# FanmingL/Recurrent-Offpolicy-RL

Hardware: AMD Instinct MI355X
Metric: env-steps/sec trained (higher is better)
Workload: dtype f32; 1 GPU; smamba_s32_c16_b2_nln SAC-REDQ update, B=64/GPU, T=1024, D=256 (configs[1]; N=8: configs[3]); row_length=1043, obs=17, act=6, critic=efc-8, global_rows=64, parallelism=dp1

## Files before the change

include/resel_hip.h:

```cpp
#ifndef RESEL_HIP_H
#define RESEL_HIP_H

#include <stddef.h>
#include <stdint.h>

#ifdef __cplusplus
extern "C" {
#endif

#define RESEL_OK 0
#define RESEL_EINVAL (-1)
#define RESEL_ELAUNCH (-2)

typedef void* resel_stream_t;

int resel_abi_version(void);
const char* resel_build_info(void);

enum {
    RESEL_PROF_SSCAN_FWD = 0, RESEL_PROF_SSCAN_BWD = 1, RESEL_PROF_ATTN_FWD = 2, RESEL_PROF_ATTN_DQ = 3, RESEL_PROF_ATTN_DKV = 4,
    RESEL_PROF_LINREC_REAL_FWD = 5, RESEL_PROF_LINREC_REAL_BWD = 6, RESEL_PROF_LINREC_COMPLEX_FWD = 7, RESEL_PROF_LINREC_COMPLEX_BWD = 8,
    RESEL_PROF_GRU_FWD = 9, RESEL_PROF_GRU_BWD = 10, RESEL_PROF_CONV_FWD = 11, RESEL_PROF_CONV_BWD = 12, RESEL_PROF_GEMM = 13,
    RESEL_PROF_SSCAN_FWD_LOCAL = 14, RESEL_PROF_SSCAN_BWD_LOCAL = 15,
    RESEL_PROF_NSLOTS = 16
// ... 230 lines not shown
#define RESEL_CATEGORICAL_MAX_ACTIONS 4096
int resel_categorical_step(const float* logits, int64_t ld_logits, const float* u, float floor, float* logp, int64_t ld_logp,
                           float* mode, float* sample, int64_t ld_idx, int M, int A, resel_stream_t stream);

#define RESEL_TMAZE_STATE_WORDS 8
typedef struct { int32_t corridor_length, oracle_length, episode_length; double goal_reward, penalty, distract_reward; } resel_tmaze_cfg_t;
int resel_tmaze_step(resel_tmaze_cfg_t cfg, int init, const float* action, int64_t ld_action, const int32_t* goals, int64_t ld_goals,
                     const int32_t* n_episodes, int J, int32_t* env_state, double* ret_acc, double* ep_ret, int32_t* ep_len,
                     int64_t ld_ep, float* in_block, int64_t ld_in, int A, int32_t* flags, int B, resel_stream_t stream);

typedef struct { int32_t state, last_state, last_action, action, next_state, reward, logp, mask, start, done, reward_input, timeout; } resel_collect_layout_t;
int resel_tmaze_collect_step(resel_tmaze_cfg_t cfg, resel_collect_layout_t lay, int init, const float* action, int64_t ld_action,
                             const int32_t* goal, int32_t* env_state, double* ret_acc, float* traj, int T_cap, int64_t ld_row,
                             int max_episode_steps, float* in_block, int64_t ld_in, int A, int B, resel_stream_t stream);

int resel_categorical_fwd(const float* logits, float floor, float* logp, float* probs, float* mode, int M, int A, resel_stream_t stream);
int resel_categorical_bwd(const float* logits, float floor, const float* dlogp, const float* dprobs, float* dlogits, int M, int A,
                          resel_stream_t stream);
int resel_discrete_value(const float* q, const int32_t* subset, int m, const float* logp, const float* log_alpha, float* v,
                         int E, int M, int A, resel_stream_t stream);
int resel_q_taken_loss_fwd(const float* q, const float* action, const float* y, const float* mask, float* out2, void* workspace,
                           int E, int M, int A, resel_stream_t stream);
int resel_q_taken_loss_bwd(const float* q, const float* action, const float* y, const float* mask, const float* g, float* dq,
                           int E, int M, int A, resel_stream_t stream);
int resel_discrete_actor_loss_fwd(const float* logp, const float* q, const float* mask, const float* log_alpha, float* out2,
                                  void* workspace, int E, int M, int A, int reduce_min, resel_stream_t stream);
int resel_discrete_actor_loss_bwd(const float* logp, const float* q, const float* mask, const float* log_alpha, const float* g,
                                  float* dlogp, float* dq, int E, int M, int A, int reduce_min, resel_stream_t stream);

size_t resel_atb_workspace_bytes(int64_t K, int Wd, int Nd);
int resel_atb(const float* wide, int64_t ldw, int Wd, const float* narrow, int64_t ldn, int Nd, float* out, int transposed,
              void* workspace, int64_t K, resel_stream_t stream);

#ifdef __cplusplus
}
#endif
#endif
```

recurrent-offpolicy-rl_amd/csrc/skinny_gemm.hip:

```cpp
#include "resel_common.h"

namespace {
using namespace resel;

typedef float f32x16 __attribute__((ext_vector_type(16)));

__device__ __forceinline__ int acc_row(int r, int half) { return (r >> 2) * 8 + half * 4 + (r & 3); }

template <int NT>
__global__ __launch_bounds__(256) void atb_kernel(const float* __restrict__ Wm, int64_t ldw, int Wd, const float* __restrict__ Nm,
                                                  int64_t ldn, int Nd, float* __restrict__ part, int64_t K, int rows_per,
                                                  int transposed) {
    const int lane = threadIdx.x & 63, wave = threadIdx.x >> 6;
    const int half = lane >> 5, col = lane & 31;
    const int wb = blockIdx.y * 512 + wave * 128;
    if (wb >= Wd) return;
    const int64_t k0 = (int64_t)blockIdx.x * rows_per;
    const int64_t k1 = k0 + rows_per < K ? k0 + rows_per : K;
    f32x16 acc[4][NT];
#pragma unroll
    for (int e = 0; e < 4; ++e)
#pragma unroll
        for (int t = 0; t < NT; ++t)
#pragma unroll
            for (int r = 0; r < 16; ++r) acc[e][t][r] = 0.f;
    const int wc = wb + 4 * col;
    const bool w_ok = wc < Wd;
    bool n_ok[NT];
#pragma unroll
    for (int t = 0; t < NT; ++t) n_ok[t] = 32 * t + col < Nd;
    constexpr int UN = NT == 1 ? 8 : 4;
    for (int64_t k = k0; k < k1; k += 2 * UN) {
// ... 2 lines not shown
#pragma unroll
        for (int u = 0; u < UN; ++u) {
            const int64_t kr = k + 2 * u + half;
            const bool ok = kr < k1;
            a[u] = (ok && w_ok) ? ld4(Wm + kr * ldw + wc) : make_float4(0.f, 0.f, 0.f, 0.f);
#pragma unroll
            for (int t = 0; t < NT; ++t) b[u][t] = (ok && n_ok[t]) ? Nm[kr * ldn + 32 * t + col] : 0.f;
        }
#pragma unroll
        for (int u = 0; u < UN; ++u)
#pragma unroll
            for (int t = 0; t < NT; ++t) {
                acc[0][t] = __builtin_amdgcn_mfma_f32_32x32x2f32(a[u].x, b[u][t], acc[0][t], 0, 0, 0);
                acc[1][t] = __builtin_amdgcn_mfma_f32_32x32x2f32(a[u].y, b[u][t], acc[1][t], 0, 0, 0);
                acc[2][t] = __builtin_amdgcn_mfma_f32_32x32x2f32(a[u].z, b[u][t], acc[2][t], 0, 0, 0);
                acc[3][t] = __builtin_amdgcn_mfma_f32_32x32x2f32(a[u].w, b[u][t], acc[3][t], 0, 0, 0);
            }
    }
    float* dst = part + (int64_t)blockIdx.x * Wd * Nd;
#pragma unroll
    for (int e = 0; e < 4; ++e)
#pragma unroll
        for (int t = 0; t < NT; ++t) {
            const int n = 32 * t + col;
            if (n >= Nd) continue;
#pragma unroll
            for (int r = 0; r < 16; ++r) {
                const int w = wb + 4 * acc_row(r, half) + e;
                if (w < Wd) dst[transposed ? (int64_t)n * Wd + w : (int64_t)w * Nd + n] = acc[e][t][r];
            }
        }
}

inline int pick_ksplit(int64_t K, int Wd, int Nd) {
    int64_t ks = (int64_t)(16 << 20) / ((int64_t)Wd * Nd * 4);
    if (ks > 512) ks = 512;
    if (ks < 32) ks = 32;
    if (ks > (K + 1) / 2) ks = (K + 1) / 2;
    return (int)(ks < 1 ? 1 : ks);
}

}

extern "C" {

size_t resel_atb_workspace_bytes(int64_t K, int Wd, int Nd) {
    return (size_t)pick_ksplit(K, Wd, Nd) * Wd * Nd * sizeof(float);
}

int resel_atb(const float* wide, int64_t ldw, int Wd, const float* narrow, int64_t ldn, int Nd, float* out, int transposed,
              void* workspace, int64_t K, resel_stream_t stream) {
    if (!wide || !narrow || !out || !workspace || K <= 0 || Wd <= 0 || Nd <= 0) return RESEL_EINVAL;
    if (Nd > 96 || (Wd & 3) || (ldw & 3) || !aligned16(wide)) return RESEL_EINVAL;
    const int ks = pick_ksplit(K, Wd, Nd);
    int rows_per = (int)((K + ks - 1) / ks);
    rows_per += rows_per & 1;
    const int nsplit = (int)((K + rows_per - 1) / rows_per);
    const dim3 grid(nsplit, (Wd + 511) / 512), block(256);
    hipStream_t s = (hipStream_t)stream;
    float* part = (float*)workspace;
    const int NT = (Nd + 31) / 32;
    switch (NT) {
        case 1: hipLaunchKernelGGL(atb_kernel<1>, grid, block, 0, s, wide, ldw, Wd, narrow, ldn, Nd, part, K, rows_per, transposed); break;
        case 2: hipLaunchKernelGGL(atb_kernel<2>, grid, block, 0, s, wide, ldw, Wd, narrow, ldn, Nd, part, K, rows_per, transposed); break;
        default: hipLaunchKernelGGL(atb_kernel<3>, grid, block, 0, s, wide, ldw, Wd, narrow, ldn, Nd, part, K, rows_per, transposed); break;
    }
    launch_colsum(part, (int64_t)Wd * Nd, nsplit, Wd * Nd, out, s);
    return launch_status();
}

}
```

recurrent-offpolicy-rl_amd/offpolicy_rnn/hip/_lib.py:

```python
import ctypes
import os
from ctypes import c_float, c_int, c_int64, c_size_t, c_uint64, c_void_p

_HERE = os.path.dirname(os.path.abspath(__file__))
LIB_PATH = os.environ.get('RESEL_HIP_LIBRARY') or os.path.join(_HERE, 'libresel_hip.so')
ABI_VERSION = 11
_lib = None

P, I, L, F, S, U = c_void_p, c_int, c_int64, c_float, c_void_p, c_uint64
E = ctypes.c_uint

RESET_MAX_SEGS, RESET_MAX_COUNTERS = 16, 8


class ResetSeg(ctypes.Structure):
    _fields_ = [('base', c_void_p), ('row_stride', c_int64), ('width', ctypes.c_int32)]


class ResetSegs(ctypes.Structure):
    _fields_ = [('seg', ResetSeg * RESET_MAX_SEGS)]


class ResetCounters(ctypes.Structure):
    _fields_ = [('pos', c_void_p * RESET_MAX_COUNTERS)]
# ... 72 lines not shown
    'resel_soft_update': (c_int, [P, P, F, L, S]),
    'resel_adamw_flat': (c_int, [P, P, P, P, L, P, P, P, I, F, F, F, I, P, S]),
    'resel_adamw_flat_bc': (c_int, [P, P, P, P, L, P, P, P, I, F, F, F, F, F, P, S]),
    'resel_adamw_flat_dev': (c_int, [P, P, P, P, L, P, P, P, I, F, F, F, P, P, S]),
    'resel_sumsq_workspace_bytes': (c_size_t, [L]),
    'resel_sumsq': (c_int, [P, L, P, P, S]),
    'resel_bias_act_fwd': (c_int, [P, P, L, I, L, I, S]),
    'resel_bias_act_bwd_workspace_bytes': (c_size_t, [L, I, L]),
    'resel_bias_act_bwd': (c_int, [P, L, P, L, P, P, P, L, I, L, I, P, E, S]),
    'resel_ensemble_head_fwd': (c_int, [P, P, P, P, P, L, I, L, S]),
    'resel_ensemble_head_bwd_workspace_bytes': (c_size_t, [L, I, L]),
    'resel_ensemble_head_bwd': (c_int, [P, P, P, P, P, P, P, L, I, L, P, E, S]),
    'resel_gemm_f32_workspace_bytes': (c_size_t, [I, I, I, I]),
    'resel_gemm_f32': (c_int, [P, L, L, I, P, L, L, I, P, L, I, P, L, L, P, I, I, I, I, I, S]),
    'resel_gemm_f32x': (c_int, [P, L, L, I, P, L, L, I, P, L, I, P, L, L, P, I, I, I, I, I, P, P, P, E, S]),
    'resel_amax_segments': (c_int, [P, P, P, I, P, E, S]),
    'resel_amax_state_bytes': (c_size_t, []),
    'resel_amax': (c_int, [P, L, L, I, I, I, P, E, P, S]),
    'resel_gemm_f32_fused_supported': (c_int, [I, I, I, I, L, L]),
    'resel_gemm_f32_fused_workspace_bytes': (c_size_t, [I, I, I, I, I]),
    'resel_gemm_f32_dact': (c_int, [P, L, L, I, P, L, L, I, P, L, L, P, L, L, P, P, I, I, I, I, P, P, P, E, S]),
    'resel_gemm_f32_head': (c_int, [P, L, L, I, P, L, L, I, P, L, P, L, P, P, L, L, P, P, I, I, I, I, P, P, P, E, S]),
    'resel_amax_check': (c_int, [P, L, L, I, I, I, P, P, I, S]),
    'resel_gemm_bf16_workspace_bytes': (c_size_t, [I, I, I]),
    'resel_gemm_bf16': (c_int, [P, L, I, I, P, L, I, I, P, P, L, I, P, I, I, I, S]),
    'resel_colsum_bf16_workspace_bytes': (c_size_t, [I, I]),
    'resel_colsum_bf16': (c_int, [P, L, I, I, P, P, S]),
    'resel_gather_trajs': (c_int, [P, I, L, P, I, I, I, I, I, I, I, I, I, P, I, P, S]),
    'resel_gather_trajs_sel': (c_int, [P, I, L, P, I, I, I, I, I, I, I, I, I, P, I, P, I, P, S]),
    'resel_mamba_conv_step': (c_int, [P, L, P, L, P, L, L, L, I, P, P, P, I, I, I, I, S]),
    'resel_selective_state_update': (c_int, [P, L, P, L, P, P, L, P, P, P, P, P, L, P, I, I, I, I, S]),
    'resel_atb_workspace_bytes': (c_size_t, [L, I, I]),
    'resel_atb': (c_int, [P, L, I, P, L, I, P, I, P, L, S]),
    'resel_attn_decode': (c_int, [P, L, P, P, I, P, P, F, I, I, I, I, S]),
    'resel_attn_decode_rows': (c_int, [P, L, P, P, P, P, F, I, I, I, I, S]),
    'resel_step_state_reset': (c_int, [P, I, ResetSegs, I, ResetCounters, I, S]),
    'resel_categorical_step': (c_int, [P, L, P, F, P, L, P, P, L, I, I, S]),
    'resel_tmaze_step': (c_int, [TMazeCfg, I, P, L, P, L, P, I, P, P, P, P, L, P, L, I, P, I, S]),
    'resel_tmaze_collect_step': (c_int, [TMazeCfg, CollectLayout, I, P, L, P, P, P, P, I, L, I, P, L, I, I, S]),
    'resel_categorical_fwd': (c_int, [P, F, P, P, P, I, I, S]),
    'resel_categorical_bwd': (c_int, [P, F, P, P, P, I, I, S]),
    'resel_discrete_value': (c_int, [P, P, I, P, P, P, I, I, I, S]),
    'resel_q_taken_loss_fwd': (c_int, [P, P, P, P, P, P, I, I, I, S]),
    'resel_q_taken_loss_bwd': (c_int, [P, P, P, P, P, P, I, I, I, S]),
    'resel_discrete_actor_loss_fwd': (c_int, [P, P, P, P, P, P, I, I, I, I, S]),
    'resel_discrete_actor_loss_bwd': (c_int, [P, P, P, P, P, P, P, I, I, I, I, S]),
}


class ReselHipUnavailable(RuntimeError):
    pass


def lib():
    global _lib
    if _lib is not None:
        return _lib
    if not os.path.exists(LIB_PATH):
        raise ReselHipUnavailable(
            f'RESeL-HIP: {LIB_PATH} not found. The MI355X kernels are the only implementation of the hot path; '
            f'build them with `python -c "import __graft_entry__ as g; g.build()"` (or `make -C recurrent-offpolicy-rl_amd/csrc`).')
    handle = ctypes.CDLL(LIB_PATH)
    for name, (res, args) in SIGNATURES.items():
        fn = getattr(handle, name, None)
        if fn is None:
            raise ReselHipUnavailable(f'RESeL-HIP: symbol {name} missing from {LIB_PATH} (stale build?)')
# ... 13 lines not shown
```

recurrent-offpolicy-rl_amd/offpolicy_rnn/hip/ops.py:

```python
import ctypes
import os
from typing import Optional

import torch

from ._lib import check, lib


def _need_cuda(name, *ts):
    for t in ts:
        if t is not None and not t.is_cuda:
            raise RuntimeError(f'RESeL-HIP: {name} needs CUDA tensors (got a {t.device} tensor); the HIP kernels are the '
                               f'only implementation of this op - there is no CPU fallback.')


def _p(t: Optional[torch.Tensor]):
    return None if t is None else ctypes.c_void_p(t.data_ptr())


if hasattr(torch._C, '_cuda_getCurrentRawStream') and hasattr(torch._C, '_cuda_getDevice'):
    def _stream():
        return ctypes.c_void_p(torch._C._cuda_getCurrentRawStream(torch._C._cuda_getDevice()))
else:
    def _stream():
# ... 57 lines not shown
        SSCAN_TIME_SEGMENTS, amax_out, epoch, _stream()), 'selective_scan_fwd')


def _sscan_bwd(Bsz, L, u, delta, z, A, Bm, Cm, D, delta_bias, start, dout, ck, du, ddelta, dz, dB, dC, dA, dD, dbias, softplus,
               amax_dz=None, amax_ddelta=None, epoch=0):
    Di, N = A.shape
    ws = _ws(lib().resel_selective_scan_bwd_workspace_bytes(Bsz, L, Di, N, SSCAN_TIME_SEGMENTS), u.device)
    check(lib().resel_selective_scan_bwd(
        _p(u), u.stride(-2), _p(delta), delta.stride(-2), _p(z), 0 if z is None else z.stride(-2), _p(A),
        _p(Bm), Bm.stride(-2), _p(Cm), Cm.stride(-2), _p(D), _p(delta_bias), _p(start),
        _p(dout), dout.stride(-2), _p(ck),
        _p(du), du.stride(-2), _p(ddelta), ddelta.stride(-2), _p(dz), 0 if dz is None else dz.stride(-2),
        _p(dB), dB.stride(-2), _p(dC), dC.stride(-2), _p(dA), _p(dD), _p(dbias), _p(ws),
        Bsz, L, Di, N, softplus, SSCAN_TIME_SEGMENTS, amax_dz, amax_ddelta, epoch, _stream()), 'selective_scan_bwd')


def _conv_fwd(Bsz, L, x, w, bias, mask, y, act, amax_y=None, epoch=0):
    Di, K = w.shape
    check(lib().resel_causal_conv1d_fwd(_p(x), x.stride(-2), _p(w), _p(bias), _p(mask), _p(y), y.stride(-2), Bsz, L, Di, K, act,
                                        amax_y, epoch, _stream()), 'causal_conv1d_fwd')


def _conv_bwd(Bsz, L, x, w, bias, mask, dy, dy2, dx, dw, db, act, amax_dx=None, epoch=0):
    Di, K = w.shape
    ws = _ws(lib().resel_causal_conv1d_bwd_workspace_bytes(Bsz, L, Di, K), x.device)
    check(lib().resel_causal_conv1d_bwd2(_p(x), x.stride(-2), _p(w), _p(bias), _p(mask), _p(dy), dy.stride(-2),
                                         _p(dy2), 0 if dy2 is None else dy2.stride(-2), _p(dx), dx.stride(-2), _p(dw), _p(db), _p(ws),
                                         Bsz, L, Di, K, act, amax_dx, epoch, _stream()), 'causal_conv1d_bwd')


class SelectiveScanFn(torch.autograd.Function):

    @staticmethod
    def forward(ctx, u, delta, A, Bm, Cm, D, z, delta_bias, start, delta_softplus, return_last_state):
        _need_cuda('selective_scan', u, delta, A, Bm, Cm)
        u, delta, Bm, Cm = _tok_major(u), _tok_major(delta), _tok_major(Bm), _tok_major(Cm)
        z = None if z is None else _tok_major(z)
        A = A.float().contiguous()
        D = None if D is None else D.float().contiguous()
        delta_bias = None if delta_bias is None else delta_bias.float().contiguous()
        Bsz, L, Di = u.shape
        N = A.shape[1]
        start = _flags(start, Bsz, L)
        out = torch.empty(Bsz, L, Di, dtype=torch.float32, device=u.device)
        need_grad = any(ctx.needs_input_grad)
        ck = None
        if need_grad:
            ck = _ws(lib().resel_selective_scan_ckpt_bytes(Bsz, L, Di, N), u.device)
        last = torch.empty(Bsz, Di, N, dtype=torch.float32, device=u.device) if return_last_state else None
        _sscan_fwd(Bsz, L, u, delta, z, A, Bm, Cm, D, delta_bias, start, out, ck, last, int(bool(delta_softplus)))
        ctx.save_for_backward(u, delta, A, Bm, Cm, D, z, delta_bias, start, ck)
        ctx.softplus = bool(delta_softplus)
        if return_last_state:
            ctx.mark_non_differentiable(last)
            return out, last
        return out

    @staticmethod
    def backward(ctx, dout, *_):
        u, delta, A, Bm, Cm, D, z, delta_bias, start, ck = ctx.saved_tensors
        Bsz, L, Di = u.shape
        N = A.shape[1]
        dout = _tok_major(dout)
        dev = u.device
        du = torch.empty(Bsz, L, Di, dtype=torch.float32, device=dev)
        ddelta = torch.empty_like(du)
        dz = torch.empty_like(du) if z is not None else None
        dB = torch.empty(Bsz, L, N, dtype=torch.float32, device=dev)
        dC = torch.empty_like(dB)
        dA = torch.empty(Di, N, dtype=torch.float32, device=dev)
        dD = torch.empty(Di, dtype=torch.float32, device=dev) if D is not None else None
        dbias = torch.empty(Di, dtype=torch.float32, device=dev) if delta_bias is not None else None
        _sscan_bwd(Bsz, L, u, delta, z, A, Bm, Cm, D, delta_bias, start, dout, ck, du, ddelta, dz, dB, dC, dA, dD, dbias, int(ctx.softplus))
        return du, ddelta, dA, dB, dC, dD, dz, dbias, None, None, None


def selective_scan_tm(u, delta, A, Bm, Cm, D=None, z=None, delta_bias=None, start=None, delta_softplus=True,
                      return_last_state=False):
    return SelectiveScanFn.apply(u, delta, A, Bm, Cm, D, z, delta_bias, start, delta_softplus, return_last_state)


def selective_scan_fn(u, delta, A, B, C, start, D=None, z=None, delta_bias=None, delta_softplus=False,
                      return_last_state=False):
    tm = lambda t: None if t is None else t.transpose(1, 2)
    st = None if start is None else start[:, 0, :]
    res = selective_scan_tm(tm(u), tm(delta), A, tm(B), tm(C), D, tm(z), delta_bias, st, delta_softplus, return_last_state)
    if return_last_state:
        return res[0].transpose(1, 2), res[1]
    return res.transpose(1, 2)




class MambaInnerFn(torch.autograd.Function):

    @staticmethod
    def forward(ctx, x, in_w, conv_w, conv_b, xproj_w, dt_w, dt_b, A_log, D, out_w, mask, start):
        _need_cuda('mamba_inner', x, in_w, conv_w, xproj_w, dt_w, A_log, out_w)
        Bsz, L, Dm = x.shape
        Di, N = A_log.shape
        R = dt_w.shape[1]
        K = conv_w.shape[-1]
        M = Bsz * L
        x2 = x.reshape(M, Dm)
        maskf, startf = _flags(mask, Bsz, L), _flags(start, Bsz, L)
        xz = mm_nt(x2, in_w)
        ctx.ax = amax_of(x2)
        cw = conv_w.reshape(Di, K).contiguous()
        xc = torch.empty(M, Di, dtype=torch.float32, device=x.device)
        track = amax_tracking() and M * Di >= (1 << 20)
        h_xc, p_xc, e_xc = _slot_args(track, x.device)
        _conv_fwd(Bsz, L, xz, cw, conv_b, maskf, xc, 1, p_xc, e_xc)
        tag_amax(xc, h_xc)
        x_dbl = mm_nt(xc, xproj_w)
        if R < 32 <= R + 2 * N and os.environ.get('RESEL_DT_PAD', '1') != '0' and gemm_split() == 2:
            w32 = place_blocks(Di, 32, [(0, 0)], dt_w.detach())
            dt = gemm_f32(x_dbl[:, :32], w32, True, True, dt_b, GEMM_SOFTPLUS, amax_a=amax_of(x_dbl), amax_b=weight_amax(dt_w))
        else:
            dt = gemm_f32(x_dbl[:, :R], dt_w, True, True, dt_b, GEMM_SOFTPLUS)
        A = A_log.float().contiguous()
        need_grad = any(ctx.needs_input_grad)
        ck = _ws(lib().resel_selective_scan_ckpt_bytes(Bsz, L, Di, N), x.device) if need_grad else None
        y = torch.empty(M, Di, dtype=torch.float32, device=x.device)
        h_y, p_y, e_y = _slot_args(track, x.device)
        _sscan_fwd(Bsz, L, xc, dt, xz[:, Di:], A, x_dbl[:, R:R + N], x_dbl[:, R + N:], D, None, startf, y, ck, None, 6, p_y, e_y)
        tag_amax(y, h_y)
        out = mm_nt(y, out_w)
        ctx.handles = keep_handles(ctx.ax, h_xc, h_y)
        ctx.save_for_backward(x2, in_w, cw, conv_b, xproj_w, dt_w, dt_b, A, D, out_w, maskf, startf, xz, xc, x_dbl, dt, y, ck)
        ctx.dims = (Bsz, L, Dm, Di, N, R, K, conv_w.shape)
        return out.view(Bsz, L, -1)

    @staticmethod
    def backward(ctx, dout):
        (x2, in_w, cw, conv_b, xproj_w, dt_w, dt_b, A, D, out_w, maskf, startf, xz, xc, x_dbl, dt, y, ck) = ctx.saved_tensors
        Bsz, L, Dm, Di, N, R, K, cw_shape = ctx.dims
        M = Bsz * L
        dev = x2.device
        do2 = dout.reshape(M, -1)
        if not do2.is_contiguous():
            do2 = do2.contiguous()
        ax, h_xc, h_y = live_handles(ctx.handles)
        d_out_w = wgrad(do2, y, amax_x=h_y)
        dy = mm_nn(do2, out_w)
        dxz = torch.empty(M, 2 * Di, dtype=torch.float32, device=dev)
        dx_dbl = torch.empty(M, R + 2 * N, dtype=torch.float32, device=dev)
        dxc = torch.empty(M, Di, dtype=torch.float32, device=dev)
        ddt = torch.empty(M, Di, dtype=torch.float32, device=dev)
        dA = torch.empty(Di, N, dtype=torch.float32, device=dev)
        dD = torch.empty(Di, dtype=torch.float32, device=dev)
        ddt_b = torch.empty(Di, dtype=torch.float32, device=dev)
        track = amax_tracking() and M * Di >= (1 << 20)
        h_dxz, p_dxz, e_b = _slot_args(track, dev)
        h_ddt, p_ddt, _ = _slot_args(track, dev)
        _sscan_bwd(Bsz, L, xc, dt, xz[:, Di:], A, x_dbl[:, R:R + N], x_dbl[:, R + N:], D, None, startf, dy, ck,
                   dxc, ddt, dxz[:, Di:], dx_dbl[:, R:R + N], dx_dbl[:, R + N:], dA, dD, ddt_b, 6, p_dxz, p_ddt, e_b)
        tag_amax(ddt, h_ddt)
        d_dt_w = atb(ddt, x_dbl[:, :R]) if R <= 32 and Di % 4 == 0 and ddt.stride(1) == 1 and ddt.stride(0) % 4 == 0 \
            else gemm_f32(ddt, x_dbl[:, :R], False, False)
        mm_nn(ddt, dt_w, out=dx_dbl[:, :R])
        d_xproj_w = wgrad(dx_dbl, xc, amax_x=h_xc)
        gx = mm_nn(dx_dbl, xproj_w)
        dcw = torch.empty(Di, K, dtype=torch.float32, device=dev)
        dcb = torch.empty(Di, dtype=torch.float32, device=dev) if conv_b is not None else None
        _conv_bwd(Bsz, L, xz, cw, conv_b, maskf, dxc, gx, dxz, dcw, dcb, 1, p_dxz, e_b)
        tag_amax(dxz, h_dxz)
        d_in_w = wgrad(dxz, x2, amax_x=ax)
        dx = mm_nn(dxz, in_w).view(Bsz, L, Dm) if ctx.needs_input_grad[0] else None
        return (dx, d_in_w, dcw.reshape(cw_shape), dcb, d_xproj_w, d_dt_w, ddt_b, dA, dD, d_out_w, None, None)


def mamba_inner_fn(x, in_w, conv_w, conv_b, xproj_w, dt_w, dt_b, A_log, D, out_w, mask=None, start=None):
    return MambaInnerFn.apply(x.float().contiguous(), in_w, conv_w, conv_b, xproj_w, dt_w, dt_b, A_log, D, out_w, mask, start)


class CausalConv1dFn(torch.autograd.Function):
    @staticmethod
    def forward(ctx, x, weight, bias, mask, activation):
        _need_cuda('causal_conv1d', x, weight)
        x = _tok_major(x)
        Bsz, L, Di = x.shape
        w = weight.float().reshape(Di, -1).contiguous()
        bias = None if bias is None else bias.float().contiguous()
        mask = _flags(mask, Bsz, L)
        y = torch.empty(Bsz, L, Di, dtype=torch.float32, device=x.device)
        _conv_fwd(Bsz, L, x, w, bias, mask, y, int(bool(activation)))
        ctx.save_for_backward(x, w, bias, mask)
        ctx.act = bool(activation)
        ctx.wshape = weight.shape
        return y

    @staticmethod
    def backward(ctx, dy):
        x, w, bias, mask = ctx.saved_tensors
        Bsz, L, Di = x.shape
        K = w.shape[1]
        dy = _tok_major(dy)
        dx = torch.empty(Bsz, L, Di, dtype=torch.float32, device=x.device)
        dw = torch.empty(Di, K, dtype=torch.float32, device=x.device)
        db = torch.empty(Di, dtype=torch.float32, device=x.device) if bias is not None else None
        _conv_bwd(Bsz, L, x, w, bias, mask, dy, None, dx, dw, db, int(ctx.act))
        return dx, dw.reshape(ctx.wshape), db, None, None


def causal_conv1d_fn(x, weight, bias=None, mask=None, activation=True):
    return CausalConv1dFn.apply(x, weight, bias, mask, activation)
# ... 1069 lines not shown

def mm_nn(g2, w, out=None):
    return gemm_f32(_unit(g2), _unit(w), True, False, out=out)


def wgrad(gy, x2, amax_x=None):
    return gemm_f32(_unit(gy), _unit(x2), False, False, amax_b=amax_x)


@torch.no_grad()
def gather_trajs(buffer, segments, max_len, skip, rows, row_len, c_mask, c_start, c_done, c_timeout, pre_pairs, sel=None):
    _need_cuda('gather_trajs', buffer, segments, pre_pairs, *(() if sel is None else (sel,)))
    assert buffer.dtype == torch.float32 and buffer.is_contiguous() and segments.dtype == torch.int32 and segments.is_contiguous()
    assert sel is None or (sel.dtype == torch.int32 and sel.dim() == 1 and sel.is_contiguous())
    W = buffer.shape[1]
    out = torch.empty(rows, row_len, W + 3, dtype=torch.float32, device=buffer.device)
    check(lib().resel_gather_trajs_sel(_p(buffer), W, buffer.shape[0], _p(segments), segments.shape[0], int(max_len), int(skip), int(rows),
                                       int(row_len), int(c_mask), int(c_start), int(c_done), int(c_timeout), _p(pre_pairs), pre_pairs.shape[0],
                                       None if sel is None else _p(sel), 0 if sel is None else sel.numel(), _p(out), _stream()), 'gather_trajs')
    return out


@torch.no_grad()
def atb(wide, narrow, transposed=False):
    _need_cuda('atb', wide, narrow)
    K, Wd = wide.shape
    Nd = narrow.shape[1]
    assert narrow.shape[0] == K and wide.stride(1) == 1 and narrow.stride(1) == 1
    out = torch.empty((Nd, Wd) if transposed else (Wd, Nd), dtype=torch.float32, device=wide.device)
    ws = _ws(lib().resel_atb_workspace_bytes(K, Wd, Nd), wide.device)
    check(lib().resel_atb(_p(wide), wide.stride(0), Wd, _p(narrow), narrow.stride(0), Nd, _p(out), int(bool(transposed)), _p(ws), K,
                          _stream()), 'atb')
    return out


@torch.no_grad()
def gemm_bf16(A, B, a_kcontig=True, b_kcontig=True, bias=None, out_dtype=torch.bfloat16, round_out=False):
    _need_cuda('gemm_bf16', A, B)
    assert A.dim() == 2 and B.dim() == 2 and A.stride(-1) == 1 and B.stride(-1) == 1
    assert A.dtype in (torch.float32, torch.bfloat16) and B.dtype in (torch.float32, torch.bfloat16)
    M, K = (A.shape[0], A.shape[1]) if a_kcontig else (A.shape[1], A.shape[0])
    N = B.shape[0] if b_kcontig else B.shape[1]
    assert (B.shape[1] if b_kcontig else B.shape[0]) == K
    out = torch.empty((M, N), dtype=out_dtype, device=A.device)
    L = lib()
    ws = _ws(L.resel_gemm_bf16_workspace_bytes(M, N, K), A.device)
    check(L.resel_gemm_bf16(_p(A), A.stride(0), int(a_kcontig), int(A.dtype == torch.bfloat16), _p(B), B.stride(0), int(b_kcontig),
                            int(B.dtype == torch.bfloat16), _p(bias), _p(out), out.stride(0), 1 if out_dtype == torch.bfloat16 else (2 if round_out else 0), _p(ws),
                            M, N, K, _stream()), 'gemm_bf16')
    return out


def gemm_bf16_ok(x, w):
    return (x.is_cuda and x.dim() == 2 and x.stride(-1) == 1 and x.dtype in (torch.float32, torch.bfloat16) and w.dtype == torch.float32
            and w.is_contiguous())


@torch.no_grad()
def colsum_bf16(x):
    M, N = x.shape
    if not (x.is_cuda and x.dtype == torch.bfloat16 and x.stride(1) == 1 and N % 8 == 0 and N <= 2048 and x.stride(0) % 8 == 0
            and x.data_ptr() % 16 == 0 and M >= 256):
        return torch.sum(x, 0, dtype=torch.float32)
    out = torch.empty(N, dtype=torch.float32, device=x.device)
    ws = _ws(lib().resel_colsum_bf16_workspace_bytes(M, N), x.device)
    check(lib().resel_colsum_bf16(_p(x), x.stride(0), M, N, _p(out), _p(ws), _stream()), 'colsum_bf16')
# ... 562 lines not shown
```

Measured before the change: 3.048 million env-steps/s.

## Add narrow-K and fused narrow-N pair kernels for Mamba dt projection

Adds a register-resident-weight MFMA kernel for GEMMs with a small K (the dt projection, with fused bias and softplus) and a fused backward kernel that computes both dX and dW from one pass over the gradient for small-N shapes. Both are wired into MambaInnerFn and on by default. The fused backward replaces the separate atb and mm_nn launches and reads ddt once instead of twice. It also skips saving the scan checkpoint when grad mode is off. The risks are extra code paths and a polynomial ELU approximation.

```diff
diff --git a/include/resel_hip.h b/include/resel_hip.h
--- a/include/resel_hip.h
+++ b/include/resel_hip.h
@@ -286,6 +286,12 @@
 int resel_atb(const float* wide, int64_t ldw, int Wd, const float* narrow, int64_t ldn, int Nd, float* out, int transposed,
               void* workspace, int64_t K, resel_stream_t stream);
 
+int resel_narrow_k(const float* A, int64_t lda, const float* W, int64_t ldw, const float* bias, float* C, int64_t ldc, int64_t M, int N,
+                   int K, int act, void* amax_out, unsigned amax_epoch, resel_stream_t stream);
+size_t resel_narrow_n_pair_workspace_bytes(int64_t M, int Wd, int Nn);
+int resel_narrow_n_pair(const float* G, int64_t ldg, int Wd, const float* W, int64_t ldw, const float* X, int64_t ldx, int Nn, float* dX,
+                        int64_t lddx, float* dW, void* workspace, int64_t M, resel_stream_t stream);
+
 #ifdef __cplusplus
 }
 #endif
diff --git a/recurrent-offpolicy-rl_amd/csrc/skinny_gemm.hip b/recurrent-offpolicy-rl_amd/csrc/skinny_gemm.hip
--- a/recurrent-offpolicy-rl_amd/csrc/skinny_gemm.hip
+++ b/recurrent-offpolicy-rl_amd/csrc/skinny_gemm.hip
@@ -1,3 +1,4 @@
+#include <type_traits>
 #include "resel_common.h"
 
 namespace {
@@ -66,6 +67,271 @@
         }
 }
 
+typedef float f32x4 __attribute__((ext_vector_type(4)));
+
+__device__ __forceinline__ float2 ld2(const float* p) { return *reinterpret_cast<const float2*>(p); }
+
+__device__ __forceinline__ float elu_acc(float x) {
+    float p = 1.f / 362880.f;
+    p = __builtin_fmaf(p, x, 1.f / 40320.f);
+    p = __builtin_fmaf(p, x, 1.f / 5040.f);
+    p = __builtin_fmaf(p, x, 1.f / 720.f);
+    p = __builtin_fmaf(p, x, 1.f / 120.f);
+    p = __builtin_fmaf(p, x, 1.f / 24.f);
+    p = __builtin_fmaf(p, x, 1.f / 6.f);
+    p = __builtin_fmaf(p, x, 0.5f);
+    p = __builtin_fmaf(p, x, 1.f);
+    const float neg = x > -0.5f ? p * x : fast_exp(x) - 1.f;
+    return x > 0.f ? x : neg;
+}
+
+template <int KQ, int ACT>
+__global__ __launch_bounds__(256) void narrow_k_kernel(const float* __restrict__ A, int64_t lda, const float* __restrict__ W, int64_t ldw,
+                                                       const float* __restrict__ bias, float* __restrict__ C, int64_t ldc, int64_t M, int N,
+                                                       int K, int wn, int64_t ntiles, AmaxOut amax) {
+    const int lane = threadIdx.x & 63, wave = threadIdx.x >> 6;
+    const int half = lane >> 5, col = lane & 31;
+    const int cw = wave & (wn - 1), tw = wave / wn, TW = 4 / wn;
+    const int nb = (blockIdx.y * wn + cw) * 128;
+    if (nb >= N) return;
+    const int n0 = nb + 4 * col;
+    const bool n_ok = n0 < N;
+    const int nr = n_ok ? n0 : 0;
+    int kc[KQ];
+#pragma unroll
+    for (int q = 0; q < KQ; ++q) kc[q] = (4 * q < K ? 4 * q : 0) + 2 * half;
+    float2 wr[KQ][4];
+#pragma unroll
+    for (int q = 0; q < KQ; ++q)
+#pragma unroll
+        for (int e = 0; e < 4; ++e) {
+            const float2 w = ld2(W + (int64_t)(nr + e) * ldw + kc[q]);
+            wr[q][e] = (n_ok && 4 * q < K) ? w : make_float2(0.f, 0.f);
+        }
+    float4 bv = make_float4(0.f, 0.f, 0.f, 0.f);
+    if (bias != nullptr) {
+        bv = make_float4(bias[nr], bias[nr + 1], bias[nr + 2], bias[nr + 3]);
+        if (!n_ok) bv = make_float4(0.f, 0.f, 0.f, 0.f);
+    }
+    float mx = 0.f;
+    int64_t tile = (int64_t)blockIdx.x * TW + tw;
+    const int64_t tstep = (int64_t)gridDim.x * TW;
+    float2 a[KQ];
+    {
+        int64_t t = tile * 32 + col;
+        t = t < M ? t : M - 1;
+#pragma unroll
+        for (int q = 0; q < KQ; ++q) a[q] = ld2(A + t * lda + kc[q]);
+    }
+    auto do_tile = [&](auto masked_tag) {
+        constexpr bool MASKED = decltype(masked_tag)::value;
+        float2 an[KQ];
+        {
+            int64_t t = (tile + tstep) * 32 + col;
+            t = t < M ? t : M - 1;
+#pragma unroll
+            for (int q = 0; q < KQ; ++q) an[q] = ld2(A + t * lda + kc[q]);
+        }
+        f32x16 acc[4];
+#pragma unroll
+        for (int e = 0; e < 4; ++e)
+#pragma unroll
+            for (int r = 0; r < 16; ++r) acc[e][r] = 0.f;
+#pragma unroll
+        for (int q = 0; q < KQ; ++q) {
+#pragma unroll
+            for (int e = 0; e < 4; ++e) acc[e] = __builtin_amdgcn_mfma_f32_32x32x2f32(a[q].x, wr[q][e].x, acc[e], 0, 0, 0);
+#pragma unroll
+            for (int e = 0; e < 4; ++e) acc[e] = __builtin_amdgcn_mfma_f32_32x32x2f32(a[q].y, wr[q][e].y, acc[e], 0, 0, 0);
+        }
+#pragma unroll
+        for (int r = 0; r < 16; ++r) {
+            const int64_t row = tile * 32 + acc_row(r, half);
+            float4 v = make_float4(acc[0][r] + bv.x, acc[1][r] + bv.y, acc[2][r] + bv.z, acc[3][r] + bv.w);
+            if (ACT == 3) v = make_float4(softplus_nb(v.x), softplus_nb(v.y), softplus_nb(v.z), softplus_nb(v.w));
+            if (ACT == 1) v = make_float4(elu_acc(v.x), elu_acc(v.y), elu_acc(v.z), elu_acc(v.w));
+            if (!MASKED || (row < M && n_ok)) {
+                st4(C + row * ldc + n0, v);
+                mx = amax4(mx, v);
+            }
+        }
+#pragma unroll
+        for (int q = 0; q < KQ; ++q) a[q] = an[q];
+    };
+    if (nb + 128 <= N && (tile + 1) * 32 <= M) {
+        do_tile(std::false_type{});
+        for (tile += tstep; (tile + 1) * 32 <= M; tile += tstep) do_tile(std::false_type{});
+    }
+    for (; tile < ntiles; tile += tstep) do_tile(std::true_type{});
+    amax_publish_wave(mx, amax);
+}
+
+template <int NT, bool DX, bool DW>
+__global__ __launch_bounds__(256) void narrow_n_pair_kernel(const float* __restrict__ G, int64_t ldg, int Wd, const float* __restrict__ Wm,
+                                                            int64_t ldw, const float* __restrict__ X, int64_t ldx, int Nn,
+                                                            float* __restrict__ dX, int64_t lddx, float* __restrict__ part, int64_t M,
+                                                            int rows_per) {
+    __shared__ float s_g[DX ? 4 : 1][16][132];
+    __shared__ float s_px[DX ? 2 : 1][4][16][16 * NT];
+    const int lane = threadIdx.x & 63, wave = threadIdx.x >> 6;
+    const int i16 = lane & 15, kq = lane >> 4;
+    const int wb = wave * 128;
+    if (!DX && wb >= Wd) return;
+    const int64_t k0 = (int64_t)blockIdx.x * rows_per;
+    const int64_t k1 = k0 + rows_per < M ? k0 + rows_per : M;
+    const int nblk = (int)((k1 - k0 + 15) / 16);
+    bool n_ok[NT], w_ok[2];
+#pragma unroll
+    for (int t = 0; t < NT; ++t) n_ok[t] = 16 * t + i16 < Nn;
+#pragma unroll
+    for (int h = 0; h < 2; ++h) w_ok[h] = wb + 64 * h + 4 * i16 < Wd;
+    int nc[NT], gc[2];
+#pragma unroll
+    for (int t = 0; t < NT; ++t) nc[t] = n_ok[t] ? 16 * t + i16 : 0;
+#pragma unroll
+    for (int h = 0; h < 2; ++h) gc[h] = w_ok[h] ? wb + 64 * h + 4 * i16 : 0;
+    const float4 zero4 = make_float4(0.f, 0.f, 0.f, 0.f);
+    const bool fast = wb + 128 <= Wd && Nn == 16 * NT && ((k1 - k0) & 15) == 0;
+    float wr[DX ? 8 : 1][4][NT];
+    auto load_w = [&](auto fast_tag) {
+        constexpr bool FAST = decltype(fast_tag)::value;
+#pragma unroll
+        for (int q = 0; q < 8; ++q)
+#pragma unroll
+            for (int c = 0; c < 4; ++c) {
+                const int w = wb + 16 * q + 4 * kq + c;
+#pragma unroll
+                for (int t = 0; t < NT; ++t) {
+                    const float v = Wm[(int64_t)(FAST || w < Wd ? w : 0) * ldw + nc[t]];
+                    wr[q][c][t] = (FAST || (w < Wd && n_ok[t])) ? v : 0.f;
+                }
+            }
+    };
+    if (DX) {
+        if (fast) load_w(std::true_type{});
+        else load_w(std::false_type{});
+    }
+    f32x4 accW[2][4][NT];
+#pragma unroll
+    for (int h = 0; h < 2; ++h)
+#pragma unroll
+        for (int e = 0; e < 4; ++e)
+#pragma unroll
+            for (int t = 0; t < NT; ++t) accW[h][e][t] = f32x4{0.f, 0.f, 0.f, 0.f};
+    float4 g[4][2];
+    float xb[4][NT];
+    auto load_block = [&](auto fast_tag, int64_t m0, float4 (&gd)[4][2], float (&xd)[4][NT]) {
+        constexpr bool FAST = decltype(fast_tag)::value;
+#pragma unroll
+        for (int s = 0; s < 4; ++s) {
+            const int64_t m = m0 + 4 * s + kq, mr = m < k1 ? m : k1 - 1;
+#pragma unroll
+            for (int h = 0; h < 2; ++h) {
+                const float4 v = ld4(G + mr * ldg + gc[h]);
+                gd[s][h] = (FAST || (m < k1 && w_ok[h])) ? v : zero4;
+            }
+#pragma unroll
+            for (int t = 0; t < NT; ++t) {
+                const float v = DW ? X[mr * ldx + nc[t]] : 0.f;
+                xd[s][t] = (FAST || (m < k1 && n_ok[t])) ? v : 0.f;
+            }
+        }
+    };
+    if (fast) load_block(std::true_type{}, k0, g, xb);
+    else load_block(std::false_type{}, k0, g, xb);
+    auto do_block = [&](auto fast_tag, int b) {
+        constexpr bool FAST = decltype(fast_tag)::value;
+        const int64_t m0 = k0 + 16 * (int64_t)b;
+        float4 gn[4][2];
+        float xn[4][NT];
+        load_block(fast_tag, m0 + 16, gn, xn);
+        if (DW) {
+#pragma unroll
+            for (int s = 0; s < 4; ++s)
+#pragma unroll
+                for (int h = 0; h < 2; ++h)
+#pragma unroll
+                    for (int t = 0; t < NT; ++t) {
+                        accW[h][0][t] = __builtin_amdgcn_mfma_f32_16x16x4f32(g[s][h].x, xb[s][t], accW[h][0][t], 0, 0, 0);
+                        accW[h][1][t] = __builtin_amdgcn_mfma_f32_16x16x4f32(g[s][h].y, xb[s][t], accW[h][1][t], 0, 0, 0);
+                        accW[h][2][t] = __builtin_amdgcn_mfma_f32_16x16x4f32(g[s][h].z, xb[s][t], accW[h][2][t], 0, 0, 0);
+                        accW[h][3][t] = __builtin_amdgcn_mfma_f32_16x16x4f32(g[s][h].w, xb[s][t], accW[h][3][t], 0, 0, 0);
+                    }
+        }
+        if (DX) {
+            float (*sg)[132] = s_g[DX ? wave : 0];
+#pragma unroll
+            for (int s = 0; s < 4; ++s)
+#pragma unroll
+                for (int h = 0; h < 2; ++h) st4(&sg[4 * s + kq][64 * h + 4 * i16], g[s][h]);
+            __builtin_amdgcn_fence(__ATOMIC_RELEASE, "wavefront");
+            __builtin_amdgcn_wave_barrier();
+            __builtin_amdgcn_fence(__ATOMIC_ACQUIRE, "wavefront");
+            f32x4 accX[NT], accY[NT];
+#pragma unroll
+            for (int t = 0; t < NT; ++t) accX[t] = accY[t] = f32x4{0.f, 0.f, 0.f, 0.f};
+#pragma unroll
+            for (int q = 0; q < 8; q += 2) {
+                const float4 a = ld4(&sg[i16][16 * q + 4 * kq]);
+                const float4 c = ld4(&sg[i16][16 * q + 16 + 4 * kq]);
+#pragma unroll
+                for (int t = 0; t < NT; ++t) {
+                    accX[t] = __builtin_amdgcn_mfma_f32_16x16x4f32(a.x, wr[q][0][t], accX[t], 0, 0, 0);
+                    accY[t] = __builtin_amdgcn_mfma_f32_16x16x4f32(c.x, wr[q + 1][0][t], accY[t], 0, 0, 0);
+                    accX[t] = __builtin_amdgcn_mfma_f32_16x16x4f32(a.y, wr[q][1][t], accX[t], 0, 0, 0);
+                    accY[t] = __builtin_amdgcn_mfma_f32_16x16x4f32(c.y, wr[q + 1][1][t], accY[t], 0, 0, 0);
+                    accX[t] = __builtin_amdgcn_mfma_f32_16x16x4f32(a.z, wr[q][2][t], accX[t], 0, 0, 0);
+                    accY[t] = __builtin_amdgcn_mfma_f32_16x16x4f32(c.z, wr[q + 1][2][t], accY[t], 0, 0, 0);
+                    accX[t] = __builtin_amdgcn_mfma_f32_16x16x4f32(a.w, wr[q][3][t], accX[t], 0, 0, 0);
+                    accY[t] = __builtin_amdgcn_mfma_f32_16x16x4f32(c.w, wr[q + 1][3][t], accY[t], 0, 0, 0);
+                }
+            }
+#pragma unroll
+            for (int t = 0; t < NT; ++t) accX[t] += accY[t];
+            float (*px)[16][16 * NT] = s_px[DX ? (b & 1) : 0];
+#pragma unroll
+            for (int t = 0; t < NT; ++t)
+#pragma unroll
+                for (int r = 0; r < 4; ++r) px[wave][4 * kq + r][16 * t + i16] = accX[t][r];
+            __syncthreads();
+            const int row = threadIdx.x >> 4, nn = threadIdx.x & 15;
+#pragma unroll
+            for (int t = 0; t < NT; ++t) {
+                const int n = 16 * t + nn;
+                if (FAST || (n < Nn && m0 + row < k1))
+                    dX[(m0 + row) * lddx + n] = ((px[0][row][n] + px[1][row][n]) + px[2][row][n]) + px[3][row][n];
+            }
+        }
+#pragma unroll
+        for (int s = 0; s < 4; ++s) {
+#pragma unroll
+            for (int h = 0; h < 2; ++h) g[s][h] = gn[s][h];
+#pragma unroll
+            for (int t = 0; t < NT; ++t) xb[s][t] = xn[s][t];
+        }
+    };
+    if (fast) {
+        do_block(std::true_type{}, 0);
+        for (int b = 1; b < nblk; ++b) do_block(std::true_type{}, b);
+    } else {
+        for (int b = 0; b < nblk; ++b) do_block(std::false_type{}, b);
+    }
+    if (DW) {
+        float* dst = part + (int64_t)blockIdx.x * Wd * Nn;
+#pragma unroll
+        for (int h = 0; h < 2; ++h)
+#pragma unroll
+            for (int e = 0; e < 4; ++e)
+#pragma unroll
+                for (int t = 0; t < NT; ++t)
+#pragma unroll
+                    for (int r = 0; r < 4; ++r) {
+                        const int w = wb + 64 * h + 4 * (4 * kq + r) + e;
+                        if (w < Wd && n_ok[t]) dst[(int64_t)w * Nn + 16 * t + i16] = accW[h][e][t][r];
+                    }
+    }
+}
+
 inline int pick_ksplit(int64_t K, int Wd, int Nd) {
     int64_t ks = (int64_t)(16 << 20) / ((int64_t)Wd * Nd * 4);
     if (ks > 512) ks = 512;
@@ -74,6 +340,19 @@
     return (int)(ks < 1 ? 1 : ks);
 }
 
+inline int pair_rows_per(int64_t M, int Wd, int Nn) {
+    const int ks = pick_ksplit(M, Wd, Nn);
+    const int64_t r = (M + ks - 1) / ks;
+    return (int)((r + 15) / 16 * 16);
+}
+template <int NT>
+void launch_pair(dim3 grid, hipStream_t s, bool dx, bool dw, const float* G, int64_t ldg, int Wd, const float* Wm, int64_t ldw, const float* X,
+                 int64_t ldx, int Nn, float* dX, int64_t lddx, float* part, int64_t M, int rows_per) {
+    const dim3 block(256);
+    if (dx && dw) hipLaunchKernelGGL((narrow_n_pair_kernel<NT, true, true>), grid, block, 0, s, G, ldg, Wd, Wm, ldw, X, ldx, Nn, dX, lddx, part, M, rows_per);
+    else if (dx) hipLaunchKernelGGL((narrow_n_pair_kernel<NT, true, false>), grid, block, 0, s, G, ldg, Wd, Wm, ldw, X, ldx, Nn, dX, lddx, part, M, rows_per);
+    else hipLaunchKernelGGL((narrow_n_pair_kernel<NT, false, true>), grid, block, 0, s, G, ldg, Wd, Wm, ldw, X, ldx, Nn, dX, lddx, part, M, rows_per);
+}
 }
 
 extern "C" {
@@ -103,4 +382,56 @@
     return launch_status();
 }
 
-}
+int resel_narrow_k(const float* A, int64_t lda, const float* W, int64_t ldw, const float* bias, float* C, int64_t ldc, int64_t M, int N,
+                   int K, int act, void* amax_out, unsigned amax_epoch, resel_stream_t stream) {
+    if (!A || !W || !C || M <= 0 || N <= 0 || K < 4 || K > 48 || (K & 3) || (N & 3)) return RESEL_EINVAL;
+    if (act != 0 && act != 1 && act != 3) return RESEL_EINVAL;
+    if ((lda & 1) || (ldw & 1) || (ldc & 3) || lda < K || ldw < K || ldc < N) return RESEL_EINVAL;
+    if ((reinterpret_cast<uintptr_t>(A) & 7u) || (reinterpret_cast<uintptr_t>(W) & 7u) || !aligned16(C)) return RESEL_EINVAL;
+    const int nchunks = (N + 127) / 128;
+    const int wn = nchunks >= 4 ? 4 : (nchunks >= 2 ? 2 : 1);
+    const int gy = (nchunks + wn - 1) / wn;
+    const int64_t ntiles = (M + 31) / 32;
+    const int64_t iters = (ntiles + 4 / wn - 1) / (4 / wn);
+    const int slots = 256 * (K <= 16 ? 2 : 1);
+    const int64_t maxwg = gy >= slots ? 1 : slots / gy;
+    const dim3 grid((unsigned)(iters < maxwg ? iters : maxwg), gy), block(256);
+    hipStream_t s = (hipStream_t)stream;
+    const AmaxOut ao{(unsigned long long*)amax_out, amax_epoch};
+#define RESEL_NK_LAUNCH(KQ, ACT) \
+    hipLaunchKernelGGL((narrow_k_kernel<KQ, ACT>), grid, block, 0, s, A, lda, W, ldw, bias, C, ldc, M, N, K, wn, ntiles, ao)
+#define RESEL_NK_ACT(KQ) \
+    do { if (act == 3) RESEL_NK_LAUNCH(KQ, 3); else if (act == 1) RESEL_NK_LAUNCH(KQ, 1); else RESEL_NK_LAUNCH(KQ, 0); } while (0)
+    if (K <= 16) RESEL_NK_ACT(4);
+    else if (K <= 32) RESEL_NK_ACT(8);
+    else RESEL_NK_ACT(12);
+#undef RESEL_NK_ACT
+#undef RESEL_NK_LAUNCH
+    return launch_status();
+}
+
+size_t resel_narrow_n_pair_workspace_bytes(int64_t M, int Wd, int Nn) {
+    return (size_t)pick_ksplit(M, Wd, Nn) * Wd * Nn * sizeof(float);
+}
+
+int resel_narrow_n_pair(const float* G, int64_t ldg, int Wd, const float* W, int64_t ldw, const float* X, int64_t ldx, int Nn, float* dX,
+                        int64_t lddx, float* dW, void* workspace, int64_t M, resel_stream_t stream) {
+    if (!G || M <= 0 || Wd <= 0 || Wd > 512 || (Wd & 3) || Nn <= 0 || Nn > 48 || (ldg & 3) || ldg < Wd || !aligned16(G)) return RESEL_EINVAL;
+    if (!dX && !dW) return RESEL_EINVAL;
+    if (dX && (!W || ldw < Nn || lddx < Nn)) return RESEL_EINVAL;
+    if (dW && (!X || !workspace || ldx < Nn)) return RESEL_EINVAL;
+    const int rows_per = pair_rows_per(M, Wd, Nn);
+    const int nsplit = (int)((M + rows_per - 1) / rows_per);
+    const dim3 grid(nsplit);
+    hipStream_t s = (hipStream_t)stream;
+    float* part = (float*)workspace;
+    switch ((Nn + 15) / 16) {
+        case 1: launch_pair<1>(grid, s, dX != nullptr, dW != nullptr, G, ldg, Wd, W, ldw, X, ldx, Nn, dX, lddx, part, M, rows_per); break;
+        case 2: launch_pair<2>(grid, s, dX != nullptr, dW != nullptr, G, ldg, Wd, W, ldw, X, ldx, Nn, dX, lddx, part, M, rows_per); break;
+        default: launch_pair<3>(grid, s, dX != nullptr, dW != nullptr, G, ldg, Wd, W, ldw, X, ldx, Nn, dX, lddx, part, M, rows_per); break;
+    }
+    if (dW) launch_colsum(part, (int64_t)Wd * Nn, nsplit, Wd * Nn, dW, s);
+    return launch_status();
+}
+
+}
diff --git a/recurrent-offpolicy-rl_amd/offpolicy_rnn/hip/_lib.py b/recurrent-offpolicy-rl_amd/offpolicy_rnn/hip/_lib.py
--- a/recurrent-offpolicy-rl_amd/offpolicy_rnn/hip/_lib.py
+++ b/recurrent-offpolicy-rl_amd/offpolicy_rnn/hip/_lib.py
@@ -128,6 +128,9 @@
     'resel_selective_state_update': (c_int, [P, L, P, L, P, P, L, P, P, P, P, P, L, P, I, I, I, I, S]),
     'resel_atb_workspace_bytes': (c_size_t, [L, I, I]),
     'resel_atb': (c_int, [P, L, I, P, L, I, P, I, P, L, S]),
+    'resel_narrow_k': (c_int, [P, L, P, L, P, P, L, L, I, I, I, P, E, S]),
+    'resel_narrow_n_pair_workspace_bytes': (c_size_t, [L, I, I]),
+    'resel_narrow_n_pair': (c_int, [P, L, I, P, L, P, L, I, P, L, P, P, L, S]),
     'resel_attn_decode': (c_int, [P, L, P, P, I, P, P, F, I, I, I, I, S]),
     'resel_attn_decode_rows': (c_int, [P, L, P, P, P, P, F, I, I, I, I, S]),
     'resel_step_state_reset': (c_int, [P, I, ResetSegs, I, ResetCounters, I, S]),
diff --git a/recurrent-offpolicy-rl_amd/offpolicy_rnn/hip/ops.py b/recurrent-offpolicy-rl_amd/offpolicy_rnn/hip/ops.py
--- a/recurrent-offpolicy-rl_amd/offpolicy_rnn/hip/ops.py
+++ b/recurrent-offpolicy-rl_amd/offpolicy_rnn/hip/ops.py
@@ -113,7 +113,7 @@
 class SelectiveScanFn(torch.autograd.Function):
 
     @staticmethod
-    def forward(ctx, u, delta, A, Bm, Cm, D, z, delta_bias, start, delta_softplus, return_last_state):
+    def forward(ctx, u, delta, A, Bm, Cm, D, z, delta_bias, start, delta_softplus, return_last_state, grad_mode=True):
         _need_cuda('selective_scan', u, delta, A, Bm, Cm)
         u, delta, Bm, Cm = _tok_major(u), _tok_major(delta), _tok_major(Bm), _tok_major(Cm)
         z = None if z is None else _tok_major(z)
@@ -124,7 +124,7 @@
         N = A.shape[1]
         start = _flags(start, Bsz, L)
         out = torch.empty(Bsz, L, Di, dtype=torch.float32, device=u.device)
-        need_grad = any(ctx.needs_input_grad)
+        need_grad = bool(grad_mode) and any(ctx.needs_input_grad)
         ck = None
         if need_grad:
             ck = _ws(lib().resel_selective_scan_ckpt_bytes(Bsz, L, Di, N), u.device)
@@ -153,12 +153,12 @@
         dD = torch.empty(Di, dtype=torch.float32, device=dev) if D is not None else None
         dbias = torch.empty(Di, dtype=torch.float32, device=dev) if delta_bias is not None else None
         _sscan_bwd(Bsz, L, u, delta, z, A, Bm, Cm, D, delta_bias, start, dout, ck, du, ddelta, dz, dB, dC, dA, dD, dbias, int(ctx.softplus))
-        return du, ddelta, dA, dB, dC, dD, dz, dbias, None, None, None
+        return du, ddelta, dA, dB, dC, dD, dz, dbias, None, None, None, None
 
 
 def selective_scan_tm(u, delta, A, Bm, Cm, D=None, z=None, delta_bias=None, start=None, delta_softplus=True,
                       return_last_state=False):
-    return SelectiveScanFn.apply(u, delta, A, Bm, Cm, D, z, delta_bias, start, delta_softplus, return_last_state)
+    return SelectiveScanFn.apply(u, delta, A, Bm, Cm, D, z, delta_bias, start, delta_softplus, return_last_state, torch.is_grad_enabled())
 
 
 def selective_scan_fn(u, delta, A, B, C, start, D=None, z=None, delta_bias=None, delta_softplus=False,
@@ -176,7 +176,7 @@
 class MambaInnerFn(torch.autograd.Function):
 
     @staticmethod
-    def forward(ctx, x, in_w, conv_w, conv_b, xproj_w, dt_w, dt_b, A_log, D, out_w, mask, start):
+    def forward(ctx, x, in_w, conv_w, conv_b, xproj_w, dt_w, dt_b, A_log, D, out_w, mask, start, grad_mode=True):
         _need_cuda('mamba_inner', x, in_w, conv_w, xproj_w, dt_w, A_log, out_w)
         Bsz, L, Dm = x.shape
         Di, N = A_log.shape
@@ -194,13 +194,15 @@
         _conv_fwd(Bsz, L, xz, cw, conv_b, maskf, xc, 1, p_xc, e_xc)
         tag_amax(xc, h_xc)
         x_dbl = mm_nt(xc, xproj_w)
-        if R < 32 <= R + 2 * N and os.environ.get('RESEL_DT_PAD', '1') != '0' and gemm_split() == 2:
+        if narrow_on() and narrow_k_ok(x_dbl[:, :R], dt_w):
+            dt = narrow_k(x_dbl[:, :R], dt_w.detach(), dt_b, GEMM_SOFTPLUS)
+        elif R < 32 <= R + 2 * N and os.environ.get('RESEL_DT_PAD', '1') != '0' and gemm_split() == 2:
             w32 = place_blocks(Di, 32, [(0, 0)], dt_w.detach())
             dt = gemm_f32(x_dbl[:, :32], w32, True, True, dt_b, GEMM_SOFTPLUS, amax_a=amax_of(x_dbl), amax_b=weight_amax(dt_w))
         else:
             dt = gemm_f32(x_dbl[:, :R], dt_w, True, True, dt_b, GEMM_SOFTPLUS)
         A = A_log.float().contiguous()
-        need_grad = any(ctx.needs_input_grad)
+        need_grad = bool(grad_mode) and any(ctx.needs_input_grad)
         ck = _ws(lib().resel_selective_scan_ckpt_bytes(Bsz, L, Di, N), x.device) if need_grad else None
         y = torch.empty(M, Di, dtype=torch.float32, device=x.device)
         h_y, p_y, e_y = _slot_args(track, x.device)
@@ -237,9 +239,12 @@
         _sscan_bwd(Bsz, L, xc, dt, xz[:, Di:], A, x_dbl[:, R:R + N], x_dbl[:, R + N:], D, None, startf, dy, ck,
                    dxc, ddt, dxz[:, Di:], dx_dbl[:, R:R + N], dx_dbl[:, R + N:], dA, dD, ddt_b, 6, p_dxz, p_ddt, e_b)
         tag_amax(ddt, h_ddt)
-        d_dt_w = atb(ddt, x_dbl[:, :R]) if R <= 32 and Di % 4 == 0 and ddt.stride(1) == 1 and ddt.stride(0) % 4 == 0 \
-            else gemm_f32(ddt, x_dbl[:, :R], False, False)
-        mm_nn(ddt, dt_w, out=dx_dbl[:, :R])
+        if narrow_on() and narrow_n_pair_ok(ddt, dt_w, x_dbl[:, :R]):
+            _, d_dt_w = narrow_n_pair(ddt, dt_w, x_dbl[:, :R], dx_out=dx_dbl[:, :R])
+        else:
+            d_dt_w = atb(ddt, x_dbl[:, :R]) if R <= 32 and Di % 4 == 0 and ddt.stride(1) == 1 and ddt.stride(0) % 4 == 0 \
+                else gemm_f32(ddt, x_dbl[:, :R], False, False)
+            mm_nn(ddt, dt_w, out=dx_dbl[:, :R])
         d_xproj_w = wgrad(dx_dbl, xc, amax_x=h_xc)
         gx = mm_nn(dx_dbl, xproj_w)
         dcw = torch.empty(Di, K, dtype=torch.float32, device=dev)
@@ -248,11 +253,12 @@
         tag_amax(dxz, h_dxz)
         d_in_w = wgrad(dxz, x2, amax_x=ax)
         dx = mm_nn(dxz, in_w).view(Bsz, L, Dm) if ctx.needs_input_grad[0] else None
-        return (dx, d_in_w, dcw.reshape(cw_shape), dcb, d_xproj_w, d_dt_w, ddt_b, dA, dD, d_out_w, None, None)
+        return (dx, d_in_w, dcw.reshape(cw_shape), dcb, d_xproj_w, d_dt_w, ddt_b, dA, dD, d_out_w, None, None, None)
 
 
 def mamba_inner_fn(x, in_w, conv_w, conv_b, xproj_w, dt_w, dt_b, A_log, D, out_w, mask=None, start=None):
-    return MambaInnerFn.apply(x.float().contiguous(), in_w, conv_w, conv_b, xproj_w, dt_w, dt_b, A_log, D, out_w, mask, start)
+    return MambaInnerFn.apply(x.float().contiguous(), in_w, conv_w, conv_b, xproj_w, dt_w, dt_b, A_log, D, out_w, mask, start,
+                              torch.is_grad_enabled())
 
 
 class CausalConv1dFn(torch.autograd.Function):
@@ -1388,6 +1394,65 @@
     check(lib().resel_atb(_p(wide), wide.stride(0), Wd, _p(narrow), narrow.stride(0), Nd, _p(out), int(bool(transposed)), _p(ws), K,
                           _stream()), 'atb')
     return out
+
+
+def narrow_on():
+    return os.environ.get('RESEL_NARROW', '1') != '0'
+
+
+def _narrow_block(t, mult, align):
+    return t.dim() == 2 and t.is_cuda and t.dtype == torch.float32 and t.stride(1) == 1 and t.stride(0) % mult == 0 \
+        and t.stride(0) >= t.shape[1] and t.data_ptr() % align == 0
+
+
+def narrow_k_ok(a, w, out=None):
+    K, N = a.shape[1], w.shape[0]
+    return 4 <= K <= 48 and K % 4 == 0 and N % 4 == 0 and a.shape[0] > 0 and w.shape[1] == K and _narrow_block(a, 2, 8) \
+        and _narrow_block(w, 2, 8) and (out is None or _narrow_block(out, 4, 16))
+
+
+@torch.no_grad()
+def narrow_k(a, w, bias=None, act=None, out=None, amax_out=None):
+    _need_cuda('narrow_k', a, w)
+    assert narrow_k_ok(a, w, out) and act != GEMM_ACCUMULATE
+    M, K = a.shape
+    N = w.shape[0]
+    if out is None:
+        out = torch.empty(M, N, dtype=torch.float32, device=a.device)
+    assert out.shape == (M, N)
+    if bias is not None:
+        bias = bias if (bias.dtype == torch.float32 and bias.is_contiguous()) else bias.float().contiguous()
+        assert bias.numel() == N
+    slot, slot_p, epoch = amax_out if amax_out is not None else (None, None, 0)
+    check(lib().resel_narrow_k(_p(a), a.stride(0), _p(w), w.stride(0), _p(bias), _p(out), out.stride(0), M, N, K, GEMM_EPILOGUES[act],
+                               slot_p, epoch, _stream()), 'narrow_k')
+    return tag_amax(out, slot)
+
+
+def narrow_n_pair_ok(g, w, x):
+    M, Wd = g.shape
+    ok = M > 0 and Wd % 4 == 0 and Wd <= 512 and _narrow_block(g, 4, 16)
+    for t, rows in ((w, Wd), (x, M)):
+        ok = ok and (t is None or (_narrow_block(t, 1, 4) and t.shape[0] == rows and 0 < t.shape[1] <= 48))
+    return ok and (w is None or x is None or w.shape[1] == x.shape[1])
+
+
+@torch.no_grad()
+def narrow_n_pair(g, w=None, x=None, dx_out=None):
+    _need_cuda('narrow_n_pair', g, w, x)
+    assert (w is not None or x is not None) and narrow_n_pair_ok(g, w, x)
+    M, Wd = g.shape
+    Nn = (w if w is not None else x).shape[1]
+    dx = dw = ws = None
+    if w is not None:
+        dx = dx_out if dx_out is not None else torch.empty(M, Nn, dtype=torch.float32, device=g.device)
+        assert dx.shape == (M, Nn) and _narrow_block(dx, 1, 4)
+    if x is not None:
+        dw = torch.empty(Wd, Nn, dtype=torch.float32, device=g.device)
+        ws = _ws(lib().resel_narrow_n_pair_workspace_bytes(M, Wd, Nn), g.device)
+    check(lib().resel_narrow_n_pair(_p(g), g.stride(0), Wd, _p(w), 0 if w is None else w.stride(0), _p(x), 0 if x is None else x.stride(0), Nn,
+                                    _p(dx), 0 if dx is None else dx.stride(0), _p(dw), _p(ws), M, _stream()), 'narrow_n_pair')
+    return dx, dw
 
 
 @torch.no_grad()
```

Measured after the change: 3.096 million env-steps/s (median of 6 runs). 1.6% higher.
